# RaikoPipe/panda-gym

Hardware: AMD Instinct MI355X
Metric: aggregate env-steps/s, PandaReach 4096 envs @1 GPU; 1/2/4/8-GPU scaling (higher is better)
Workload: dtype f32; 1 GPU; PandaReach-v3 (ee control, sparse reward), 4096 envs per GPU, the reference's scene: table / plane contacts of the robot (BASELINE configs[1]); envs_per_gpu=4096, global_envs=4096, parallelism=env-sharded x1

## Files before the change

panda-gym_amd/csrc/pgx_kernels.hip:

```cpp
#include <hip/hip_runtime.h>
#include <math.h>
#include <stdint.h>

#include "../../include/pgx.h"
#include "pgx_default_model.h"
#include "pgx_common.h"
#include "pgx_dev.h"
#include "pgx_model_consts.h"
#include "pgx_rows.h"

#ifdef PGX_PROF
#define PGX_PROF_N 24
__device__ unsigned long long pgx_prof_counters[PGX_PROF_N];
#define PGX_PROF_WAVES 16384
__device__ unsigned long long pgx_prof_wave[PGX_PROF_WAVES][10];
extern "C" int pgx_prof_wave_read(unsigned long long* out, int n) {
    return (int)hipMemcpyFromSymbol(out, HIP_SYMBOL(pgx_prof_wave), sizeof(unsigned long long) * 10 * (size_t)n);
}
extern "C" int pgx_prof_read(unsigned long long* out, int clear) {
    hipError_t e = hipMemcpyFromSymbol(out, HIP_SYMBOL(pgx_prof_counters), sizeof(unsigned long long) * PGX_PROF_N);
    if (e == hipSuccess && clear) {
        unsigned long long z[PGX_PROF_N] = {0};
        e = hipMemcpyToSymbol(HIP_SYMBOL(pgx_prof_counters), z, sizeof z);
    }
// ... 2319 lines not shown
                PGX_PROF_SWEEP();
                if (resid <= res_thr || it + 1 >= n_it) break;
                resid = 0.0f;
#pragma unroll
                for (int r = 0; r < PGX_N_ROWS; r++)
                    if ((kPgxRowCode[r] >> 4) == 0) row(r, resid);
                limit_check();
                if (CONT && any_contact) contact_rows(resid);
                PGX_PROF_SWEEP();
                if (resid <= res_thr) break;
            }
            redo = __any(lmargin < 0.0f) || e.pgs_mode == 3;
            if (redo) {
                PGX_PROF_COUNT(12, 1);
#pragma unroll
                for (int j = 0; j < NJ; j++) dv[j] = L.spec0[j][ln];
                dvl = v3(L.spec0[NJ][ln], L.spec0[NJ + 1][ln], L.spec0[NJ + 2][ln]);
                dvw = v3(L.spec0[NJ + 3][ln], L.spec0[NJ + 4][ln], L.spec0[NJ + 5][ln]);
#pragma unroll
                for (int r = 0; r < PGX_N_ROWS; r++) lam[r] = 0.0f;
#pragma unroll
                for (int k = 0; k < CG; k++)
#pragma unroll
                    for (int dir = 0; dir < 3; dir++) {
                        lam0[k][dir] = (CONT && OBJ && k < n0) ? L.g0q[k][1 + dir][ln].w : 0.0f;
                        lam1[k][dir] = (CONT && k < n1) ? L.g1q[k][dir][5][ln].w : 0.0f;
                    }
            }
        } else {
            PGX_PROF_COUNT(13, 1);
        }
        for (int it = 0; redo && it < n_it; it += 2) {
            float resid = 0.0f;
#pragma unroll
            for (int r = PGX_N_ROWS - 1; r >= 0; r--) row(r, resid);
            if (CONT && any_contact) contact_rows(resid);
            PGX_PROF_SWEEP();
            if (resid <= res_thr || it + 1 >= n_it) break;
            resid = 0.0f;
#pragma unroll
            for (int r = 0; r < PGX_N_ROWS; r++) row(r, resid);
            if (CONT && any_contact) contact_rows(resid);
            PGX_PROF_SWEEP();
            if (resid <= res_thr) break;
        }
    }
#undef MINV
    PGX_PROF_SWEEPS_DONE();
    PGX_TRAP(4, n1, dv, NJ, m);
    PGX_PROF_MARK(4);
    PGX_PROF_COUNT(11, any_contact ? 1 : 0);
#pragma unroll
    for (int j = 0; j < NJ; j++) {
        float vn = fminf(fmaxf(vu[j] + dv[j], -m.max_vel), m.max_vel);
        qd[j] = vn;
        q[j] += m.dt * vn;
    }
    PGX_TRAP(5, n1, q, NJ, m);
    PGX_TRAP(6, n1, qd, NJ, m);
    if (CONT) {
        ContactLds& L = *Lp;
#pragma unroll
        for (int s = 0; s < CG; s++) {
            L.cache[2 * s][ln] = s < n0 ? L.g0id[s][ln] : -1.0f;
            L.cache[2 * s + 1][ln] = s < n0 ? lam0[s][0] : 0.0f;
            L.cache[8 + 2 * s][ln] = s < n1 ? L.g1id[s][ln] : -1.0f;
            L.cache[8 + 2 * s + 1][ln] = s < n1 ? lam1[s][0] : 0.0f;
        }
    }
    if (OBJ) object_integrate(m, ob, vcu + dvl, wcu + dvw);
    PGX_PROF_MARK(5);
}

constexpr bool limit_rows_paired() {
    for (int r = 0; r < NJ; r++)
        if ((kPgxRowCode[r] >> 4) != 0) return false;
    for (int r = NJ; r + 1 < PGX_N_ROWS; r += 2)
        if ((kPgxRowCode[r] >> 4) != 1 || (kPgxRowCode[r + 1] >> 4) != 2 ||
            (kPgxRowCode[r] & 15) != (kPgxRowCode[r + 1] & 15))
            return false;
    return (PGX_N_ROWS - NJ) % 2 == 0;
}

template <int OBJ, int CONT, int PART = 1, int AO = 0, int FULL = 0>
__device__ __forceinline__ bool substep_g(MPtr mp, const PgxDevEnv& e, float* q, float* qd, const float* tq,
                                          ObjState& ob, ContactLdsGT<OBJ, FULL>* Lp, int es, int c, const LaneK& K,
                                          bool check = false) {
    MRef m = *fresh(mp);
    constexpr bool LDS_LIM = OBJ;
    constexpr bool NO_PART = OBJ && PART == 2;
    constexpr bool PERS = CONT && FULL && (OBJ || (AO && AO_PERS));
    Dyn D;
    substep_dyn_g<OBJ, CONT, AO, FULL>(m, e, q, qd, ob, Lp, es, D, c, K, check);
    if constexpr (AO) {
        if (D.coll) return true;
    }
    const V3 (&z)[NJ] = D.z;
    const V3 (&o)[NJ] = D.o;
    float vu[NJ];
#pragma unroll
    for (int j = 0; j < NJ; j++) vu[j] = D.vu[j];
    V3 vcu = D.vcu, wcu = D.wcu;
    PGX_PROF_MARK(2);
    const bool arm = c < NJ;
    const float inv_m = e.obj_inv_mass, inv_i = e.obj_inv_inertia;
    float mcol[NJ];
#pragma unroll
    for (int d = 0; d < NJ; d++) mcol[d] = D.mcol[d];
    const float kobj = OBJ ? ((c >= 7 && c < 10) ? inv_m : ((c >= 10 && c < 13) ? inv_i : 0.0f)) : 0.0f;
    const float vu_c = pick_gen(vu, vcu, wcu);
    float gv = 0.0f;

    constexpr int P0 = OBJ ? CG : 0;
    constexpr int CGR = ContactLdsGT<OBJ, FULL>::CGR;
    constexpr int NP = P0 + (CONT ? CGR : 0);
    constexpr int RB = CONT ? ContactLdsGT<OBJ, FULL>::RB : CGR;
    constexpr int NQR = ContactLdsGT<OBJ, FULL>::NQR;
    constexpr int NC_ = OBJ ? 13 : NJ;
    constexpr int XSTEP = 1;
    int n1x = 0;
    int nxr = 0;
    float cJ[NP > 0 ? NP : 1][3], cR[NP > 0 ? NP : 1][3], crhs[NP > 0 ? NP : 1][3], cjinv[NP > 0 ? NP : 1][3];
    float cden[NP > 0 ? NP : 1][3], clam[NP > 0 ? NP : 1][3];
    float pmu[NP > 0 ? NP : 1];
    bool act[NP > 0 ? NP : 1];
    int n0 = 0, n1 = 0;
    if (CONT) {
        ContactLdsGT<OBJ, FULL>& L = *Lp;
        n0 = L.cnt[0][es];
        n1 = L.cnt[1][es];
        const float erp_dt = m.contact_erp * m.inv_dt;
        float cid0[CG], cim0[CG], cid1[CGR], cim1[CGR];
#pragma unroll
        for (int s2 = 0; s2 < CG; s2++) {
            cid0[s2] = OBJ ? L.cache[2 * s2][es] : -1.0f;
            cim0[s2] = OBJ ? L.cache[2 * s2 + 1][es] : 0.0f;
        }
#pragma unroll
        for (int s2 = 0; s2 < CGR; s2++) {
            cid1[s2] = L.cache[CACHE1 + 2 * s2][es];
            cim1[s2] = L.cache[CACHE1 + 2 * s2 + 1][es];
        }
        auto warm_of = [&](const float* ids, const float* ims, auto n_c, float id) __attribute__((always_inline)) {
            float w = 0.0f;
#pragma unroll
            for (int s2 = 0; s2 < decltype(n_c)::value; s2++) w = ids[s2] == id ? m.warmstart * ims[s2] : w;
            return w;
        };
#pragma unroll
        for (int p = 0; p < NP; p++) pmu[p] = m.friction;
#pragma unroll
        for (int k = 0; k < P0; k++) {
            act[k] = k < n0;
            const float4 r4 = L.g0q[k][0][es];
            const V3 r = v3(r4.x, r4.y, r4.z);
            const float id = L.g0id[k][es];
            const float warm = warm_of(cid0, cim0, IC<CG>{}, id);
            V3 nk = lds3(L.g0n[k], es), t1, t2;
            nk = act[k] ? nk : v3(0.0f, 0.0f, 1.0f);
            plane_space(nk, t1, t2);
#pragma unroll
            for (int dir = 0; dir < 3; dir++) {
                const V3 lin = dir == 0 ? nk : (dir == 1 ? t1 : t2);
                const V3 ang = cross(r, lin);
                const float den = inv_m + dot(ang, ang) * inv_i;
                const float jinv = den > 2.220446e-16f ? fast_rcp(den) : 0.0f;
// ... 228 lines not shown
                    w = fmaf(Jq[l], bcast16<l>(gv), w);
                });
                gwr = w;
            };
            build(IC<0>{}, Wm, Wc, gw);
            if constexpr (TWO) { if (g1k_any[1]) build(IC<1>{}, Wm2, Wc2, gw2); }
        }
    }
    constexpr int XB = (RB > CGR) ? (3 * (RB - CGR) + GW - 1) / GW : 1;
    float xs_rhs[XB], xs_lam[XB], xs_fk[XB], xs_jinv[XB];
    auto load_xs = [&](bool start) __attribute__((always_inline)) {
        if constexpr (RB > CGR) {
            ContactLdsGT<OBJ, FULL>& L = *Lp;
            __builtin_amdgcn_fence(__ATOMIC_SEQ_CST, "wavefront");
#pragma unroll
            for (int b = 0; b < XB; b++) {
                const int xq = GW * b + c;
                const bool ok = xq < 3 * nxr;
                const int xr = ok ? xq : 0;
                xs_lam[b] = ok ? L.xlam0[xr][es] : 0.0f;
                if (start) {
                    xs_rhs[b] = ok ? L.xrhs[xr][es] : 0.0f;
                    xs_fk[b] = ok ? L.xfk[xr][es] : 0.0f;
                    xs_jinv[b] = ok ? L.xjinv[xr][es] : 0.0f;
                }
            }
        }
    };
#pragma unroll
    for (int b = 0; b < XB; b++) { xs_rhs[b] = 0.0f; xs_lam[b] = 0.0f; xs_fk[b] = 0.0f; xs_jinv[b] = 0.0f; }
    if (RB > CGR && nxr > 0) load_xs(true);
    PGX_PROF_MARK(23);

    float den[NJ], jinv[NJ];
#pragma unroll
    for (int d = 0; d < NJ; d++) {
        den[d] = D.mdiag[d];
        jinv[d] = den[d] > 2.220446e-16f ? fast_rcp(den[d]) : 0.0f;
    }
    float rhs[PGX_N_ROWS];
#pragma unroll
    for (int r = 0; r < PGX_N_ROWS; r++) {
        const int kind = kPgxRowCode[r] >> 4, d = kPgxRowCode[r] & 15;
        rhs[r] = 0.0f;
        if (kind == 0) {
            const float pos_term = (tq[d] - q[d]) * m.inv_dt;
            const float desired = m.kp * pos_term + vu[d] + m.kd * (0.0f - vu[d]);
            rhs[r] = desired - vu[d];
        }
    }
    auto init_limit_rows = [&]() __attribute__((always_inline)) {
#pragma unroll
        for (int r = 0; r < PGX_N_ROWS; r++) {
            const int kind = kPgxRowCode[r] >> 4, d = kPgxRowCode[r] & 15;
            if (kind == 0) continue;
            const float rel = kind == 2 ? -vu[d] : vu[d];
            const float pen = kind == 1 ? (q[d] - kLower[d]) : (kUpper[d] - q[d]);
            float verr = -rel, perr = 0.0f;
            if (pen > 0.0f) verr -= pen * m.inv_dt;
            else perr = -pen * m.erp * m.inv_dt;
            rhs[r] = perr + verr;
        }
    };
    bool ok_c = true;
    bool far_nc = true;
    if (arm) {
        float B = 0.0f;
#pragma unroll
        for (int k = 0; k < NJ; k++) B += fabsf(mcol[k]) * m.max_impulse[k];
        B = B * 1.001f + 1e-6f;
        float lo_a[NJ], up_a[NJ];
#pragma unroll
        for (int d = 0; d < NJ; d++) { lo_a[d] = kLower[d]; up_a[d] = kUpper[d]; }
        const float qc = pick_arm(q, 0.0f);
        const float penl = qc - pick_arm(lo_a, 0.0f), penu = pick_arm(up_a, 0.0f) - qc;
        ok_c = penl > 0.0f && penu > 0.0f && (vu_c - B) > -penl * m.inv_dt && (vu_c + B) < penu * m.inv_dt;
    }
    far_nc = !row_any(!ok_c);
    const bool far = far_nc && n1 == 0;
    float mcs[NJ], wms[NJ], wms2[NJ];
    constexpr int PK = AO ? PGX_PK_AO : PGX_PK;
    constexpr bool PKM = WROWS && (PK & 1) != 0, PKC = WROWS && (PK & 2) != 0;
    constexpr bool PKD = TWO && FULL && !PKM && !PKC && (PK & 4) != 0;
    f2 mw[NJ], crw[NQ], mw2[NJ], cw2[NQ];
    f2 bnd[NJ];
    float lam[PGX_N_ROWS], lhi[NJ];
#pragma unroll
    for (int d = 0; d < NJ; d++) {
        mcs[d] = mcol[d] * jinv[d];
        wms[d] = Wm[d] * jinv[d];
        wms2[d] = Wm2[d] * jinv[d];
        lhi[d] = m.limit_max_imp * den[d];
    }
    auto init_bounds = [&]() __attribute__((always_inline)) {
#pragma unroll
        for (int r = 0; r < PGX_N_ROWS; r++) {
            const int kind = kPgxRowCode[r] >> 4, d = kPgxRowCode[r] & 15;
            lam[r] = 0.0f;
            if (kind == 0) bnd[d] = (f2){-m.max_impulse[d] * den[d], m.max_impulse[d] * den[d]};
            else if (LDS_LIM) __hip_atomic_store(&Lp->llam[r - NJ][es], 0.0f, __ATOMIC_RELAXED, __HIP_MEMORY_SCOPE_WAVEFRONT);
        }
    };
    init_bounds();
    auto mrow = [&](auto rc, auto g2_c, float& resid) __attribute__((always_inline)) {
        constexpr int r = decltype(rc)::value;
        constexpr int kind = kPgxRowCode[r] >> 4, d = kPgxRowCode[r] & 15;
        const float x = kind == 2 ? rhs[r] + bcast16<d>(gv) : rhs[r] - bcast16<d>(gv);
        float delta;
        if constexpr (kind == 0) {
            delta = __builtin_amdgcn_fmed3f(x, bnd[d].x, bnd[d].y);
            bnd[d] -= (f2){delta, delta};
        } else if constexpr (LDS_LIM) {
            float* lr = &Lp->lrhs[r - NJ][es];
            float* ll = &Lp->llam[r - NJ][es];
            const float rr = __hip_atomic_load(lr, __ATOMIC_RELAXED, __HIP_MEMORY_SCOPE_WAVEFRONT);
            const float lm = __hip_atomic_load(ll, __ATOMIC_RELAXED, __HIP_MEMORY_SCOPE_WAVEFRONT);
            const float xl = kind == 2 ? rr + bcast16<d>(gv) : rr - bcast16<d>(gv);
            delta = __builtin_amdgcn_fmed3f(xl, -lm, lhi[d] - lm);
            __hip_atomic_store(ll, lm + delta, __ATOMIC_RELAXED, __HIP_MEMORY_SCOPE_WAVEFRONT);
        } else {
            delta = __builtin_amdgcn_fmed3f(x, -lam[r], lhi[d] - lam[r]);
            lam[r] += delta;
        }
        const float sd = kind == 2 ? -delta : delta;
        if constexpr (PKD) {
            gv += mcs[d] * sd;
            if constexpr (decltype(g2_c)::value) pk_fma_acc(gw, gw2, mw2[d], sd);
            else gw += mw2[d].x * sd;
        } else {
            if constexpr (PKM) {
                pk_fma_acc(gv, gw, mw[d], sd);
            } else {
                gv += mcs[d] * sd;
                if constexpr (WROWS) gw += wms[d] * sd;
            }
            if constexpr (TWO && decltype(g2_c)::value) gw2 += wms2[d] * sd;
        }
        resid = fmaxf(resid, fabsf(delta));
    };
    constexpr int NPP = NP > 0 ? NP : 1;
    float fk[NPP][3];
    bool rok[NPP][3];
#pragma unroll
    for (int p = 0; p < NP; p++)
#pragma unroll
        for (int dir = 0; dir < 3; dir++) {
            rok[p][dir] = act[p] && cjinv[p][dir] != 0.0f;
            fk[p][dir] = rok[p][dir] ? pmu[p] * cjinv[p][0] * cden[p][dir] : 0.0f;
            crhs[p][dir] *= cden[p][dir];
            clam[p][dir] *= cden[p][dir];
            cR[p][dir] *= cjinv[p][dir];
        }
    if constexpr (WROWS) {
#pragma unroll
        for (int q = 0; q < NQ; q++) {
            Wc[q] *= cjinv[q / 3][q % 3];
            if (TWO) Wc2[q] *= cjinv[q / 3][q % 3];
        }
        float r0 = 0.0f, r1 = 0.0f;
        sfor<0, NQ>([&](auto qc) __attribute__((always_inline)) {
            constexpr int q = decltype(qc)::value;
            if constexpr (q < GW) r0 = lane_sel<q>(crhs[q / 3][q % 3], r0);
            else r1 = lane_sel<q - GW>(crhs[q / 3][q % 3], r1);
        });
        gw = r0 - gw;
        if (TWO) gw2 = r1 - gw2;
        if constexpr (OBJ) {
            sfor<0, NQ / 3>([&](auto pc) __attribute__((always_inline)) {
                constexpr int p = decltype(pc)::value, q = 3 * p;
                const bool usable = act[p] && cjinv[p][0] != 0.0f;
                if constexpr (q < GW) gw = usable ? gw : lane_sel<q>(-3.0e38f, gw);
                else gw2 = usable ? gw2 : lane_sel<q - GW>(-3.0e38f, gw2);
            });
        }
#pragma unroll
        for (int q = 0; q < NQ; q++) { Wc[q] = -Wc[q]; Wc2[q] = -Wc2[q]; }
#pragma unroll
        for (int d = 0; d < NJ; d++) { wms[d] = -wms[d]; wms2[d] = -wms2[d]; }
        if constexpr (PKM) {
#pragma unroll
            for (int d = 0; d < NJ; d++) mw[d] = (f2){mcs[d], wms[d]};
        }
        if constexpr (PKC) {
#pragma unroll
            for (int q = 0; q < NQ; q++) crw[q] = (f2){cR[q / 3][q % 3], Wc[q]};
        }
        if constexpr (PKD) {
#pragma unroll
            for (int d = 0; d < NJ; d++) mw2[d] = (f2){wms[d], wms2[d]};
#pragma unroll
            for (int q = 0; q < NQ; q++) cw2[q] = (f2){Wc[q], Wc2[q]};
        }
    }
    float chi[NPP];
    if constexpr (CONT) {
#pragma unroll
        for (int p = 0; p < NP; p++) Lp->pjn[p][es] = cjinv[p][0];
    }
#pragma unroll
    for (int p = 0; p < NP; p++) {
        chi[p] = rok[p][0] ? 3.0e38f : 0.0f;
        if (WROWS && !rok[p][0]) clam[p][0] = 0.0f;
    }
    auto crow = [&](auto pc, auto dc, const bool fr, auto g2_c, float& resid) __attribute__((always_inline)) {
        constexpr int p = decltype(pc)::value, dir = decltype(dc)::value, q = 3 * p + dir;
        const float ln_n = clam[p][0], lm = clam[p][dir];
        float lo, hi;
        if (fr) {
            const float mk = ln_n > 0.0f ? 1.0f : 0.0f;
            const float fkv = fk[p][dir];
            const f2 b = ((f2){-fkv, fkv} * ln_n - lm) * mk;
            lo = b.x;
            hi = b.y;
        } else {
            lo = -lm;
            hi = OBJ ? 3.0e38f : chi[p];
        }
        const float x = q < GW ? bcast16<q % GW>(gw) : bcast16<q % GW>(gw2);
        const float delta = __builtin_amdgcn_fmed3f(x, lo, hi);
        clam[p][dir] = lm + delta;
        if constexpr (PKD) {
            gv += cR[p][dir] * delta;
            if constexpr (decltype(g2_c)::value) pk_fma_acc(gw, gw2, cw2[q], delta);
            else gw += cw2[q].x * delta;
        } else {
            if constexpr (PKC) {
                pk_fma_acc(gv, gw, crw[q], delta);
            } else {
                gv += cR[p][dir] * delta;
                gw += Wc[q] * delta;
            }
            if constexpr (TWO && decltype(g2_c)::value) gw2 += Wc2[q] * delta;
        }
        resid = fmaxf(resid, fabsf(delta));
    };
    int n1w = 0;
#pragma unroll
    for (int k = 0; k < CGR; k++) n1w = g1k_any[k] ? k + 1 : n1w;
    n1w = __builtin_amdgcn_readfirstlane(n1w);
    const bool g0_any = CONT && OBJ && __any(n0 > 0);
    const bool g1_any = CONT && __any(n1 > 0);
    int rcol = c;
    auto extra_rows = [&](auto fr_c, auto nx_c, auto g2_c, float& resid) __attribute__((always_inline)) {
        constexpr int FR = decltype(fr_c)::value, NX = decltype(nx_c)::value;
        if constexpr (WROWS && RB > CGR && NX > 0) {
            ContactLdsGT<OBJ, FULL>& L = *Lp;
            const float gvb = gv;
            sfor<0, NX>([&](auto kc) __attribute__((always_inline)) {
                constexpr int kx = decltype(kc)::value;
                sfor<FR ? 1 : 0, FR ? 3 : 1>([&](auto dc) __attribute__((always_inline)) {
                    constexpr int dir = decltype(dc)::value, xq = 3 * kx + dir;
                    constexpr int b = xq / GW, l = xq % GW, bn = (3 * kx) / GW, ln_ = (3 * kx) % GW;
                    const float J = L.xd[es][xq][c].x;
                    const float Rs = L.xd[es][xq][rcol].y;
                    const float w = sum16(J * gv);
                    const float lm = bcast16<l>(xs_lam[b]), fkv = bcast16<l>(xs_fk[b]);
                    float lo, hi;
                    if constexpr (dir != 0) {
                        const float ln_n = bcast16<ln_>(xs_lam[bn]);
                        const float mk = ln_n > 0.0f ? 1.0f : 0.0f;
                        const f2 bb = ((f2){-fkv, fkv} * ln_n - lm) * mk;
                        lo = bb.x;
                        hi = bb.y;
                    } else {
                        lo = -lm;
                        hi = fkv;
                    }
                    const float delta = __builtin_amdgcn_fmed3f(bcast16<l>(xs_rhs[b]) - w, lo, hi);
                    xs_lam[b] = lane_sel<l>(lm + delta, xs_lam[b]);
                    gv += Rs * delta;
                    resid = fmaxf(resid, fabsf(delta));
                });
            });
            const float dgv = gv - gvb;
            auto correct = [&](auto reg_c, float& gwr) __attribute__((always_inline)) {
                constexpr int R0 = decltype(reg_c)::value * GW;
                const int qr = R0 + c < NQR ? R0 + c : NQR - 1;
                const float4* jrow = &L.wJ[es][qr][0];
                float Jq[NC];
#pragma unroll
                for (int v4 = 0; v4 < (NC + 3) / 4; v4++) {
                    const float4 t = jrow[v4];
                    const float tv[4] = {t.x, t.y, t.z, t.w};
#pragma unroll
                    for (int u = 0; u < 4; u++)
                        if (4 * v4 + u < NC) Jq[4 * v4 + u] = tv[u];
                }
                float d = Jq[0] * bcast16<0>(dgv);
                sfor<1, NC>([&](auto lc) __attribute__((always_inline)) {
                    constexpr int l2 = decltype(lc)::value;
                    d = fmaf(Jq[l2], bcast16<l2>(dgv), d);
                });
                gwr -= R0 + c < NQR ? d : 0.0f;
            };
            correct(IC<0>{}, gw);
            if constexpr (TWO && decltype(g2_c)::value) correct(IC<1>{}, gw2);
        }
    };
    auto contact_rows = [&](auto nw_c, auto nx_c, auto g2_c, float& resid) __attribute__((always_inline)) {
        constexpr int NW = decltype(nw_c)::value;
#pragma unroll
        for (int fr = 0; fr < 2; fr++) {
            if (OBJ && g0_any) {
                sfor<0, P0>([&](auto kc) __attribute__((always_inline)) {
                    if (fr) { crow(kc, IC<1>{}, true, g2_c, resid); crow(kc, IC<2>{}, true, g2_c, resid); }
                    else crow(kc, IC<0>{}, false, g2_c, resid);
                });
            }
            if (NW < 0 && !g1_any) continue;
            sfor<0, (CONT ? (NW >= 0 ? NW : CGR) : 0)>([&](auto kc) __attribute__((always_inline)) {
                constexpr int k = decltype(kc)::value;
                if (NW >= 0 || k < n1w) {
                    if (fr) {
                        crow(IC<P0 + k>{}, IC<1>{}, true, g2_c, resid);
                        crow(IC<P0 + k>{}, IC<2>{}, true, g2_c, resid);
                    } else {
                        crow(IC<P0 + k>{}, IC<0>{}, false, g2_c, resid);
                    }
                }
            });
            if (fr) extra_rows(IC<1>{}, nx_c, g2_c, resid);
            else extra_rows(IC<0>{}, nx_c, g2_c, resid);
        }
    };
    const bool any_contact = CONT && __any(n0 > 0 || n1 > 0);
    const int n_it = m.num_iterations;
    float res_thr = m.residual_abs;
    asm("" : "+s"(res_thr));
    PGX_PROF_MARK(3);
    PGX_PROF_COUNT(9, 1);
    PGX_PROF_SWEEPS_DECL;
    float rl_c = -1.0f, ru_c = -1.0f;
    float lmargin = 3.0e38f;
    auto limit_check = [&]() __attribute__((always_inline)) {
        lmargin = fminf(lmargin, fminf(gv - rl_c, -(ru_c + gv)));
    };
    constexpr int KMAX = CONT ? 1 : 2;
    constexpr int SL0 = OBJ ? 13 : NJ;
    unsigned dmask = 0u;
    float smcs[KMAX], swms[KMAX], swms2[KMAX], srh[KMAX][2], slhi[KMAX], slam[KMAX][2];
    f2 smw[KMAX];
    auto srow = [&](auto sc, auto kc, auto g2_c, float& resid) __attribute__((always_inline)) {
        constexpr int S = decltype(sc)::value, KIND = decltype(kc)::value;
        const float x = KIND == 2 ? srh[S][1] + bcast16<SL0 + S>(gv) : srh[S][0] - bcast16<SL0 + S>(gv);
        const float delta = __builtin_amdgcn_fmed3f(x, -slam[S][KIND - 1], slhi[S] - slam[S][KIND - 1]);
        slam[S][KIND - 1] += delta;
        const float sd = KIND == 2 ? -delta : delta;
        if constexpr (PKM) {
            pk_fma_acc(gv, gw, smw[S], sd);
        } else {
            gv += smcs[S] * sd;
            if constexpr (WROWS) gw += swms[S] * sd;
        }
        if constexpr (TWO && decltype(g2_c)::value) gw2 += swms2[S] * sd;
        resid = fmaxf(resid, fabsf(delta));
    };
    static_assert(limit_rows_paired(), "limit rows come as (lower, upper) pairs of one dof after the motor rows");
    auto solve = [&](auto mode_c, auto nw_c, auto k_c, auto nx_c) __attribute__((always_inline)) {
        constexpr int MODE = decltype(mode_c)::value;
        constexpr int NW = decltype(nw_c)::value;
        constexpr int K = decltype(k_c)::value;
        constexpr bool G2 = TWO && (NW < 0 || 3 * (P0 + NW) > GW);
        const IC<G2 ? 1 : 0> g2_c{};
        for (int it = 0; it < n_it; it += 2) {
            float resid = 0.0f;
            if constexpr (MODE == 1 || MODE == 3) limit_check();
            if constexpr (MODE == 3) {
                sfor<0, K>([&](auto i) __attribute__((always_inline)) {
                    constexpr int S = K - 1 - decltype(i)::value;
                    srow(IC<S>{}, IC<2>{}, g2_c, resid);
                    srow(IC<S>{}, IC<1>{}, g2_c, resid);
                    limit_check();
                });
            }
            sfor<0, PGX_N_ROWS>([&](auto i) __attribute__((always_inline)) {
                constexpr int r = PGX_N_ROWS - 1 - decltype(i)::value;
                if constexpr (MODE == 2 || (kPgxRowCode[r] >> 4) == 0) mrow(IC<r>{}, g2_c, resid);
            });
            if (CONT && (OBJ || NW > 0 || (NW < 0 && any_contact))) contact_rows(nw_c, nx_c, g2_c, resid);
            PGX_PROF_SWEEP();
            if (resid <= res_thr || it + 1 >= n_it) break;
            resid = 0.0f;
            sfor<0, PGX_N_ROWS>([&](auto i) __attribute__((always_inline)) {
                constexpr int r = decltype(i)::value;
                if constexpr (MODE == 2 || (kPgxRowCode[r] >> 4) == 0) mrow(IC<r>{}, g2_c, resid);
            });
            if constexpr (MODE == 1 || MODE == 3) limit_check();
            if constexpr (MODE == 3) {
                sfor<0, K>([&](auto sc) __attribute__((always_inline)) {
                    srow(sc, IC<1>{}, g2_c, resid);
                    srow(sc, IC<2>{}, g2_c, resid);
                    limit_check();
                });
            }
            if (CONT && (OBJ || NW > 0 || (NW < 0 && any_contact))) contact_rows(nw_c, nx_c, g2_c, resid);
            PGX_PROF_SWEEP();
            if (resid <= res_thr) break;
        }
    };
    auto solve_w = [&](auto mode_c, auto k_c) __attribute__((always_inline)) {
        constexpr int MODE = decltype(mode_c)::value;
        if constexpr (WROWS) {
            if (n1w == 0) solve(mode_c, IC<0>{}, k_c, IC<0>{});
            else if (nxr == 0 && n1w <= 2) solve(mode_c, IC<2>{}, k_c, IC<0>{});
            else if (CGR > 4 && nxr == 0 && n1w <= 4) solve(mode_c, IC<(CGR > 4 ? 4 : CGR)>{}, k_c, IC<0>{});
            else if constexpr (RB > CGR && MODE != 3) {
                if (nxr == 0) {
                    solve(mode_c, IC<CGR>{}, k_c, IC<0>{});
                } else {
                    sfor<1, (RB - CGR) / XSTEP + 1>([&](auto ic) __attribute__((always_inline)) {
                        constexpr int NXC = decltype(ic)::value * XSTEP;
                        if (nxr == NXC) solve(mode_c, IC<CGR>{}, k_c, IC<NXC>{});
                    });
                }
            } else {
                solve(mode_c, IC<CGR>{}, k_c, IC<0>{});
            }
        } else {
            solve(mode_c, IC<-1>{}, k_c, IC<0>{});
        }
    };
#ifndef PGX_NO_PARK_SOLVE
    constexpr bool PARK_SOLVE = CONT && (OBJ || AO || PART == 2);
#else
    constexpr bool PARK_SOLVE = false;
#endif
    auto park = [&](int k, float v) __attribute__((always_inline)) {
        __hip_atomic_store(&Lp->psv[k][es], v, __ATOMIC_RELAXED, __HIP_MEMORY_SCOPE_WAVEFRONT);
    };
    auto unpark = [&](int k) __attribute__((always_inline)) {
        return __hip_atomic_load(&Lp->psv[k][es], __ATOMIC_RELAXED, __HIP_MEMORY_SCOPE_WAVEFRONT);
    };
    if constexpr (PARK_SOLVE) {
#pragma unroll
        for (int j = 0; j < NJ; j++) { park(j, q[j]); park(NJ + j, vu[j]); }
        if constexpr (OBJ) {
            park(14, ob.p.x); park(15, ob.p.y); park(16, ob.p.z);
            park(17, ob.qx); park(18, ob.qy); park(19, ob.qz); park(20, ob.qw);
            park(21, vcu.x); park(22, vcu.y); park(23, vcu.z);
            park(24, wcu.x); park(25, wcu.y); park(26, wcu.z);
        }
    }
    if (__all(far)) {
        solve(IC<0>{}, IC<0>{}, IC<0>{}, IC<0>{});
    } else {
        PGX_PROF_COUNT(10, 1);
        init_limit_rows();
        if constexpr (LDS_LIM) {
#pragma unroll
            for (int r = NJ; r < PGX_N_ROWS; r++)
                __hip_atomic_store(&Lp->lrhs[r - NJ][es], rhs[r], __ATOMIC_RELAXED, __HIP_MEMORY_SCOPE_WAVEFRONT);
        }
        if (e.pgs_mode != 2) {
            float rl[NJ], ru[NJ];
#pragma unroll
            for (int r = NJ; r < PGX_N_ROWS; r++) {
                const int kind = kPgxRowCode[r] >> 4, d = kPgxRowCode[r] & 15;
                if (kind == 1) rl[d] = rhs[r];
                else ru[d] = rhs[r];
            }
            rl_c = pick_arm(rl, -3.0e38f);
            ru_c = pick_arm(ru, -3.0e38f);
            const bool spec_all = __all(far_nc);
            int nk = 0;
            if (!spec_all) {
                const uint64_t bm = __ballot(arm && !ok_c);
                dmask = __builtin_amdgcn_readfirstlane((unsigned)((bm | (bm >> 16) | (bm >> 32) | (bm >> 48)) & 0x7Fu));
                nk = __builtin_popcount(dmask);
            }
            const float gv0 = gv, gw0 = gw, gw20 = gw2;
            if constexpr (CONT) {
#pragma unroll
                for (int p = 0; p < NP; p++) Lp->pl0[p][es] = clam[p][0];
            }
            if (PART && !NO_PART && !spec_all && nk <= KMAX && nxr == 0) {
                PGX_PROF_COUNT(7, 1);
                int ds[2] = {0, 0};
                int k = 0;
                sfor<0, (PGX_N_ROWS - NJ) / 2>([&](auto pc) __attribute__((always_inline)) {
                    constexpr int d = kPgxRowCode[NJ + 2 * decltype(pc)::value] & 15;
                    if ((dmask >> d) & 1u) { if (k == 0) ds[0] = d; else ds[1] = d; k++; }
                });
                ds[0] = __builtin_amdgcn_readfirstlane(ds[0]);
                ds[1] = __builtin_amdgcn_readfirstlane(ds[1]);
                const int src = (int)(threadIdx.x & ~(unsigned)(GW - 1));
                auto mirror = [&](float& x) __attribute__((always_inline)) {
                    x = lane_sel<SL0>(__shfl(x, src + ds[0]), x);
                    if (KMAX > 1 && nk > 1) x = lane_sel<SL0 + 1>(__shfl(x, src + ds[1]), x);
                };
#pragma unroll
                for (int d = 0; d < NJ; d++) {
                    if constexpr (PKM) {
                        float t = mw[d].x;
                        mirror(t);
                        mw[d].x = t;
                    } else {
                        mirror(mcs[d]);
                    }
                }
                mirror(gv);
                if (g1_any) {
#pragma unroll
                    for (int p = 0; p < NP; p++)
#pragma unroll
                        for (int dir = 0; dir < 3; dir++) {
                            if constexpr (PKC) {
                                float t = crw[3 * p + dir].x;
                                mirror(t);
                                crw[3 * p + dir].x = t;
                            } else {
                                mirror(cR[p][dir]);
                            }
                        }
                }
#pragma unroll
                for (int S = 0; S < KMAX; S++) {
                    if constexpr (PKM) smw[S] = mw[0];
                    else { smcs[S] = mcs[0]; swms[S] = PKD ? mw2[0].x : wms[0]; }
                    swms2[S] = PKD ? mw2[0].y : wms2[0]; slhi[S] = lhi[0];
                    srh[S][0] = rl[0]; srh[S][1] = ru[0];
                    slam[S][0] = 0.0f; slam[S][1] = 0.0f;
                    sfor<1, NJ>([&](auto dc) __attribute__((always_inline)) {
                        constexpr int d = decltype(dc)::value;
                        const bool hit = ds[S] == d;
                        auto sel = [&](float a, float o) __attribute__((always_inline)) { return hit ? a : o; };
                        if constexpr (PKM) smw[S] = hit ? mw[d] : smw[S];
                        else { smcs[S] = sel(mcs[d], smcs[S]); swms[S] = sel(PKD ? mw2[d].x : wms[d], swms[S]); }
                        swms2[S] = sel(PKD ? mw2[d].y : wms2[d], swms2[S]);
                        slhi[S] = sel(lhi[d], slhi[S]);
                        srh[S][0] = sel(rl[d], srh[S][0]); srh[S][1] = sel(ru[d], srh[S][1]);
                    });
                }
                if ((dmask >> c) & 1u) { rl_c = -3.0e38f; ru_c = -3.0e38f; }
                if (c == SL0) rcol = ds[0];
                if (KMAX > 1 && nk > 1 && c == SL0 + 1) rcol = ds[1];
                PGX_PROF_COUNT(16, nk == 2 ? 1 : 0);
                PGX_PROF_COUNT(18, any_contact ? 1 : 0);
                if (KMAX == 1 || nk == 1) solve_w(IC<3>{}, IC<1>{});
                else solve_w(IC<3>{}, IC<KMAX>{});
            } else if (spec_all) {
                solve_w(IC<1>{}, IC<0>{});
            } else {
                lmargin = -1.0f;
            }
            const bool viol = lmargin < 0.0f;
            if (__any(row_any(viol)) || e.pgs_mode == 3) {
                PGX_PROF_COUNT(12, 1);
                gv = gv0;
                gw = gw0;
                gw2 = gw20;
#pragma unroll
                for (int p = 0; p < NP; p++) {
                    clam[p][0] = CONT ? Lp->pl0[p][es] : 0.0f;
                    clam[p][1] = 0.0f;
                    clam[p][2] = 0.0f;
                }
                if (RB > CGR && nxr > 0) load_xs(false);
                init_bounds();
                solve_w(IC<2>{}, IC<0>{});
            }
        } else {
            PGX_PROF_COUNT(13, 1);
            solve_w(IC<2>{}, IC<0>{});
        }
    }
    PGX_PROF_SWEEPS_DONE();
    PGX_PROF_MARK(4);
    PGX_PROF_COUNT(11, any_contact ? 1 : 0);
    if constexpr (PARK_SOLVE) {
#pragma unroll
        for (int j = 0; j < NJ; j++) { q[j] = unpark(j); vu[j] = unpark(NJ + j); }
        if constexpr (OBJ) {
            ob.p = v3(unpark(14), unpark(15), unpark(16));
            ob.qx = unpark(17); ob.qy = unpark(18); ob.qz = unpark(19); ob.qw = unpark(20);
            vcu = v3(unpark(21), unpark(22), unpark(23));
            wcu = v3(unpark(24), unpark(25), unpark(26));
        }
    }
    sfor<0, NJ>([&](auto jc) __attribute__((always_inline)) {
        constexpr int j = decltype(jc)::value;
        const float vn = fminf(fmaxf(vu[j] + bcast16<j>(gv), -m.max_vel), m.max_vel);
        qd[j] = vn;
        q[j] += m.dt * vn;
    });
    if (CONT) {
        ContactLdsGT<OBJ, FULL>& L = *Lp;
        float gid0[CG], pj0[CG], gid1[CGR], pj1[CGR];
#pragma unroll
        for (int s = 0; s < CG; s++) {
            gid0[s] = OBJ ? L.g0id[s][es] : -1.0f;
            pj0[s] = OBJ ? L.pjn[s][es] : 0.0f;
        }
#pragma unroll
        for (int s = 0; s < CGR; s++) {
            gid1[s] = L.g1id[s][es];
            pj1[s] = L.pjn[P0 + s][es];
        }
#pragma unroll
        for (int s = 0; s < CG; s++) {
            L.cache[2 * s][es] = (OBJ && s < n0) ? gid0[s] : -1.0f;
            L.cache[2 * s + 1][es] = (OBJ && s < n0) ? clam[s][0] * pj0[s] : 0.0f;
        }
#pragma unroll
        for (int s = 0; s < CGR; s++) {
            L.cache[CACHE1 + 2 * s][es] = s < n1 ? gid1[s] : -1.0f;
            L.cache[CACHE1 + 2 * s + 1][es] = s < n1 ? clam[P0 + s][0] * pj1[s] : 0.0f;
        }
        if constexpr (RB > CGR) {
            if (n1x > CGR) {
#pragma unroll
                for (int b = 0; b < XB; b++)
                    if (GW * b + c < 3 * (n1x - CGR)) L.xlam[GW * b + c][es] = xs_lam[b];
                __builtin_amdgcn_fence(__ATOMIC_SEQ_CST, "wavefront");
            }
            for (int s = CGR; s < RB; s++) {
                const int xq = 3 * (s - CGR);
                L.cache[CACHE1 + 2 * s][es] = s < n1 ? L.g1id[s][es] : -1.0f;
                L.cache[CACHE1 + 2 * s + 1][es] = s < n1 ? L.xlam[xq][es] * L.xjinv[xq][es] : 0.0f;
            }
        }
        if constexpr (PERS) {
            static_assert(RB <= GW, "one lane per robot slot");
            __builtin_amdgcn_fence(__ATOMIC_SEQ_CST, "wavefront");
            if (c < n1) {
                const int w = L.g1w[c][es];
                if (w >= 0) L.mimp[w][es] = L.cache[CACHE1 + 2 * c + 1][es];
            }
        }
    }
    if (OBJ) {
        const V3 dvl = v3(bcast16<7>(gv), bcast16<8>(gv), bcast16<9>(gv));
        const V3 dvw = v3(bcast16<10>(gv), bcast16<11>(gv), bcast16<12>(gv));
        object_integrate(m, ob, vcu + dvl, wcu + dvw);
    }
    PGX_PROF_MARK(5);
    return false;
}

__device__ __forceinline__ void ee_state(MRef m, const float* q, const float* qd, V3& pos, V3& vel) {
    Chain k;
    fk_chain(m, q, k);
    pos = k.o[NJ - 1] + mulc(k.R[NJ - 1], kEeCom);
    V3 vv = v3(0, 0, 0);
#pragma unroll
    for (int j = 0; j < NJ; j++) vv = vv + qd[j] * cross(col(k.R[j], 2), pos - k.o[j]);
    vel = vv;
// ... 1279 lines not shown
```

Baseline: 11.20 million env-steps/s.

## Merge contact-row gradient into upper lanes of motor gradient register in PGS solve

```diff
diff --git a/panda-gym_amd/csrc/pgx_kernels.hip b/panda-gym_amd/csrc/pgx_kernels.hip
--- a/panda-gym_amd/csrc/pgx_kernels.hip
+++ b/panda-gym_amd/csrc/pgx_kernels.hip
@@ -2425,6 +2425,13 @@
     return (PGX_N_ROWS - NJ) % 2 == 0;
 }
 
+constexpr int last_motor_row() {
+    int r = 0;
+    for (int i = 0; i < PGX_N_ROWS; i++)
+        if ((kPgxRowCode[i] >> 4) == 0) r = i;
+    return r;
+}
+
 template <int OBJ, int CONT, int PART = 1, int AO = 0, int FULL = 0>
 __device__ __forceinline__ bool substep_g(MPtr mp, const PgxDevEnv& e, float* q, float* qd, const float* tq,
                                           ObjState& ob, ContactLdsGT<OBJ, FULL>* Lp, int es, int c, const LaneK& K,
@@ -2819,6 +2826,15 @@
     constexpr int PK = AO ? PGX_PK_AO : PGX_PK;
     constexpr bool PKM = WROWS && (PK & 1) != 0, PKC = WROWS && (PK & 2) != 0;
     constexpr bool PKD = TWO && FULL && !PKM && !PKC && (PK & 4) != 0;
+    constexpr bool MERGE = WROWS && !OBJ && !AO && !PKM && !PKC && PART != 2;
+    constexpr int MG0 = 8;
+    static_assert(!MERGE || MG0 + 6 <= GW, "6 contact rows from lane MG0");
+    auto hi_sel = [&](float a, float other) __attribute__((always_inline)) {
+        float r;
+        asm("v_cndmask_b32 %0, %1, %2, %3" : "=v"(r) : "v"(other), "v"(a), "s"(0xFF00FF00FF00FF00ull));
+        return r;
+    };
+    auto ror8 = [&](float v) __attribute__((always_inline)) { return dpp<0x128>(v); };
     f2 mw[NJ], crw[NQ], mw2[NJ], cw2[NQ];
     f2 bnd[NJ];
     float lam[PGX_N_ROWS], lhi[NJ];
@@ -2839,7 +2855,7 @@
         }
     };
     init_bounds();
-    auto mrow = [&](auto rc, auto g2_c, float& resid) __attribute__((always_inline)) {
+    auto mrow = [&](auto rc, auto g2_c, auto mg_c, float& resid) __attribute__((always_inline)) {
         constexpr int r = decltype(rc)::value;
         constexpr int kind = kPgxRowCode[r] >> 4, d = kPgxRowCode[r] & 15;
         const float x = kind == 2 ? rhs[r] + bcast16<d>(gv) : rhs[r] - bcast16<d>(gv);
@@ -2860,7 +2876,9 @@
             lam[r] += delta;
         }
         const float sd = kind == 2 ? -delta : delta;
-        if constexpr (PKD) {
+        if constexpr (decltype(mg_c)::value) {
+            gv += mcs[d] * sd;
+        } else if constexpr (PKD) {
             gv += mcs[d] * sd;
             if constexpr (decltype(g2_c)::value) pk_fma_acc(gw, gw2, mw2[d], sd);
             else gw += mw2[d].x * sd;
@@ -2873,7 +2891,8 @@
             }
             if constexpr (TWO && decltype(g2_c)::value) gw2 += wms2[d] * sd;
         }
-        resid = fmaxf(resid, fabsf(delta));
+        if constexpr (decltype(mg_c)::value == 2) resid = fabsf(delta);
+        else resid = fmaxf(resid, fabsf(delta));
     };
     constexpr int NPP = NP > 0 ? NP : 1;
     float fk[NPP][3];
@@ -2939,7 +2958,7 @@
         chi[p] = rok[p][0] ? 3.0e38f : 0.0f;
         if (WROWS && !rok[p][0]) clam[p][0] = 0.0f;
     }
-    auto crow = [&](auto pc, auto dc, const bool fr, auto g2_c, float& resid) __attribute__((always_inline)) {
+    auto crow = [&](auto pc, auto dc, const bool fr, auto g2_c, auto mg_c, float& resid) __attribute__((always_inline)) {
         constexpr int p = decltype(pc)::value, dir = decltype(dc)::value, q = 3 * p + dir;
         const float ln_n = clam[p][0], lm = clam[p][dir];
         float lo, hi;
@@ -2953,10 +2972,14 @@
             lo = -lm;
             hi = OBJ ? 3.0e38f : chi[p];
         }
-        const float x = q < GW ? bcast16<q % GW>(gw) : bcast16<q % GW>(gw2);
+        constexpr bool MG = decltype(mg_c)::value != 0;
+        const float x = MG ? bcast16<(MG0 + q) % GW>(gv)
+                           : (q < GW ? bcast16<q % GW>(gw) : bcast16<q % GW>(gw2));
         const float delta = __builtin_amdgcn_fmed3f(x, lo, hi);
         clam[p][dir] = lm + delta;
-        if constexpr (PKD) {
+        if constexpr (MG) {
+            gv += cR[p][dir] * delta;
+        } else if constexpr (PKD) {
             gv += cR[p][dir] * delta;
             if constexpr (decltype(g2_c)::value) pk_fma_acc(gw, gw2, cw2[q], delta);
             else gw += cw2[q].x * delta;
@@ -2969,7 +2992,8 @@
             }
             if constexpr (TWO && decltype(g2_c)::value) gw2 += Wc2[q] * delta;
         }
-        resid = fmaxf(resid, fabsf(delta));
+        if constexpr (decltype(mg_c)::value == 2) resid = fabsf(delta);
+        else resid = fmaxf(resid, fabsf(delta));
     };
     int n1w = 0;
 #pragma unroll
@@ -3034,14 +3058,14 @@
             if constexpr (TWO && decltype(g2_c)::value) correct(IC<1>{}, gw2);
         }
     };
-    auto contact_rows = [&](auto nw_c, auto nx_c, auto g2_c, float& resid) __attribute__((always_inline)) {
+    auto contact_rows = [&](auto nw_c, auto nx_c, auto g2_c, auto mg_c, float& resid) __attribute__((always_inline)) {
         constexpr int NW = decltype(nw_c)::value;
 #pragma unroll
         for (int fr = 0; fr < 2; fr++) {
             if (OBJ && g0_any) {
                 sfor<0, P0>([&](auto kc) __attribute__((always_inline)) {
-                    if (fr) { crow(kc, IC<1>{}, true, g2_c, resid); crow(kc, IC<2>{}, true, g2_c, resid); }
-                    else crow(kc, IC<0>{}, false, g2_c, resid);
+                    if (fr) { crow(kc, IC<1>{}, true, g2_c, mg_c, resid); crow(kc, IC<2>{}, true, g2_c, mg_c, resid); }
+                    else crow(kc, IC<0>{}, false, g2_c, mg_c, resid);
                 });
             }
             if (NW < 0 && !g1_any) continue;
@@ -3049,10 +3073,10 @@
                 constexpr int k = decltype(kc)::value;
                 if (NW >= 0 || k < n1w) {
                     if (fr) {
-                        crow(IC<P0 + k>{}, IC<1>{}, true, g2_c, resid);
-                        crow(IC<P0 + k>{}, IC<2>{}, true, g2_c, resid);
+                        crow(IC<P0 + k>{}, IC<1>{}, true, g2_c, mg_c, resid);
+                        crow(IC<P0 + k>{}, IC<2>{}, true, g2_c, mg_c, resid);
                     } else {
-                        crow(IC<P0 + k>{}, IC<0>{}, false, g2_c, resid);
+                        crow(IC<P0 + k>{}, IC<0>{}, false, g2_c, mg_c, resid);
                     }
                 }
             });
@@ -3074,87 +3098,119 @@
     };
     constexpr int KMAX = CONT ? 1 : 2;
     constexpr int SL0 = OBJ ? 13 : NJ;
+    static_assert(!MERGE || SL0 + KMAX <= MG0, "the slot lanes (mirror() writes SL0 .. SL0 + KMAX - 1) end below the merged contact lanes");
+    static_assert((kPgxRowCode[0] >> 4) == 0, "row 0 is a motor row (the first row of a forward sweep)");
     unsigned dmask = 0u;
     float smcs[KMAX], swms[KMAX], swms2[KMAX], srh[KMAX][2], slhi[KMAX], slam[KMAX][2];
     f2 smw[KMAX];
-    auto srow = [&](auto sc, auto kc, auto g2_c, float& resid) __attribute__((always_inline)) {
+    auto srow = [&](auto sc, auto kc, auto g2_c, auto mg_c, float& resid) __attribute__((always_inline)) {
         constexpr int S = decltype(sc)::value, KIND = decltype(kc)::value;
         const float x = KIND == 2 ? srh[S][1] + bcast16<SL0 + S>(gv) : srh[S][0] - bcast16<SL0 + S>(gv);
         const float delta = __builtin_amdgcn_fmed3f(x, -slam[S][KIND - 1], slhi[S] - slam[S][KIND - 1]);
         slam[S][KIND - 1] += delta;
         const float sd = KIND == 2 ? -delta : delta;
-        if constexpr (PKM) {
+        if constexpr (decltype(mg_c)::value) {
+            gv += smcs[S] * sd;
+        } else if constexpr (PKM) {
             pk_fma_acc(gv, gw, smw[S], sd);
         } else {
             gv += smcs[S] * sd;
             if constexpr (WROWS) gw += swms[S] * sd;
         }
         if constexpr (TWO && decltype(g2_c)::value) gw2 += swms2[S] * sd;
-        resid = fmaxf(resid, fabsf(delta));
+        if constexpr (decltype(mg_c)::value == 2) resid = fabsf(delta);
+        else resid = fmaxf(resid, fabsf(delta));
     };
     static_assert(limit_rows_paired(), "limit rows come as (lower, upper) pairs of one dof after the motor rows");
-    auto solve = [&](auto mode_c, auto nw_c, auto k_c, auto nx_c) __attribute__((always_inline)) {
+    auto solve = [&](auto mode_c, auto nw_c, auto k_c, auto nx_c, auto mg_c) __attribute__((always_inline)) {
         constexpr int MODE = decltype(mode_c)::value;
         constexpr int NW = decltype(nw_c)::value;
         constexpr int K = decltype(k_c)::value;
         constexpr bool G2 = TWO && (NW < 0 || 3 * (P0 + NW) > GW);
         const IC<G2 ? 1 : 0> g2_c{};
+        constexpr bool MG = decltype(mg_c)::value != 0;
+        const IC<MG ? 2 : 0> mgf_c{};
+        constexpr int LASTM = last_motor_row();
         for (int it = 0; it < n_it; it += 2) {
             float resid = 0.0f;
             if constexpr (MODE == 1 || MODE == 3) limit_check();
             if constexpr (MODE == 3) {
                 sfor<0, K>([&](auto i) __attribute__((always_inline)) {
                     constexpr int S = K - 1 - decltype(i)::value;
-                    srow(IC<S>{}, IC<2>{}, g2_c, resid);
-                    srow(IC<S>{}, IC<1>{}, g2_c, resid);
+                    if constexpr (MG && S == K - 1) srow(IC<S>{}, IC<2>{}, g2_c, mgf_c, resid);
+                    else srow(IC<S>{}, IC<2>{}, g2_c, mg_c, resid);
+                    srow(IC<S>{}, IC<1>{}, g2_c, mg_c, resid);
                     limit_check();
                 });
             }
             sfor<0, PGX_N_ROWS>([&](auto i) __attribute__((always_inline)) {
                 constexpr int r = PGX_N_ROWS - 1 - decltype(i)::value;
-                if constexpr (MODE == 2 || (kPgxRowCode[r] >> 4) == 0) mrow(IC<r>{}, g2_c, resid);
+                if constexpr (MG && MODE != 3 && r == LASTM) mrow(IC<r>{}, g2_c, mgf_c, resid);
+                else if constexpr (MODE == 2 || (kPgxRowCode[r] >> 4) == 0) mrow(IC<r>{}, g2_c, mg_c, resid);
             });
-            if (CONT && (OBJ || NW > 0 || (NW < 0 && any_contact))) contact_rows(nw_c, nx_c, g2_c, resid);
+            if (CONT && (OBJ || NW > 0 || (NW < 0 && any_contact))) contact_rows(nw_c, nx_c, g2_c, mg_c, resid);
             PGX_PROF_SWEEP();
             if (resid <= res_thr || it + 1 >= n_it) break;
             resid = 0.0f;
             sfor<0, PGX_N_ROWS>([&](auto i) __attribute__((always_inline)) {
                 constexpr int r = decltype(i)::value;
-                if constexpr (MODE == 2 || (kPgxRowCode[r] >> 4) == 0) mrow(IC<r>{}, g2_c, resid);
+                if constexpr (MG && r == 0) mrow(IC<r>{}, g2_c, mgf_c, resid);
+                else if constexpr (MODE == 2 || (kPgxRowCode[r] >> 4) == 0) mrow(IC<r>{}, g2_c, mg_c, resid);
             });
             if constexpr (MODE == 1 || MODE == 3) limit_check();
             if constexpr (MODE == 3) {
                 sfor<0, K>([&](auto sc) __attribute__((always_inline)) {
-                    srow(sc, IC<1>{}, g2_c, resid);
-                    srow(sc, IC<2>{}, g2_c, resid);
+                    srow(sc, IC<1>{}, g2_c, mg_c, resid);
+                    srow(sc, IC<2>{}, g2_c, mg_c, resid);
                     limit_check();
                 });
             }
-            if (CONT && (OBJ || NW > 0 || (NW < 0 && any_contact))) contact_rows(nw_c, nx_c, g2_c, resid);
+            if (CONT && (OBJ || NW > 0 || (NW < 0 && any_contact))) contact_rows(nw_c, nx_c, g2_c, mg_c, resid);
             PGX_PROF_SWEEP();
             if (resid <= res_thr) break;
         }
     };
-    auto solve_w = [&](auto mode_c, auto k_c) __attribute__((always_inline)) {
+    const bool mg = MERGE && e.pgs_mode != 4 && n1w >= 1 && n1w <= 2 && nxr == 0;
+    auto merge_rows = [&]() __attribute__((always_inline)) {
+        if constexpr (MERGE) {
+#pragma unroll
+            for (int d = 0; d < NJ; d++) mcs[d] = hi_sel(ror8(wms[d]), mcs[d]);
+#pragma unroll
+            for (int q = 0; q < 6; q++) cR[q / 3][q % 3] = hi_sel(ror8(Wc[q]), cR[q / 3][q % 3]);
+            gv = hi_sel(ror8(gw), gv);
+        }
+    };
+    auto split_rows = [&]() __attribute__((always_inline)) {
+        if constexpr (MERGE) {
+#pragma unroll
+            for (int d = 0; d < NJ; d++) wms[d] = hi_sel(0.0f, ror8(mcs[d]));
+#pragma unroll
+            for (int q = 0; q < 6; q++) Wc[q] = hi_sel(0.0f, ror8(cR[q / 3][q % 3]));
+        }
+    };
+    auto solve_w = [&](auto mode_c, auto k_c, auto mgi_c) __attribute__((always_inline)) {
         constexpr int MODE = decltype(mode_c)::value;
-        if constexpr (WROWS) {
-            if (n1w == 0) solve(mode_c, IC<0>{}, k_c, IC<0>{});
-            else if (nxr == 0 && n1w <= 2) solve(mode_c, IC<2>{}, k_c, IC<0>{});
-            else if (CGR > 4 && nxr == 0 && n1w <= 4) solve(mode_c, IC<(CGR > 4 ? 4 : CGR)>{}, k_c, IC<0>{});
+        const IC<0> m0{};
+        if constexpr (decltype(mgi_c)::value) {
+            solve(mode_c, IC<2>{}, k_c, IC<0>{}, IC<(MODE != 2) ? 1 : 0>{});
+        } else if constexpr (WROWS) {
+            if (n1w == 0) solve(mode_c, IC<0>{}, k_c, IC<0>{}, m0);
+            else if (nxr == 0 && n1w <= 2) solve(mode_c, IC<2>{}, k_c, IC<0>{}, m0);
+            else if (CGR > 4 && nxr == 0 && n1w <= 4) solve(mode_c, IC<(CGR > 4 ? 4 : CGR)>{}, k_c, IC<0>{}, m0);
             else if constexpr (RB > CGR && MODE != 3) {
                 if (nxr == 0) {
-                    solve(mode_c, IC<CGR>{}, k_c, IC<0>{});
+                    solve(mode_c, IC<CGR>{}, k_c, IC<0>{}, m0);
                 } else {
                     sfor<1, (RB - CGR) / XSTEP + 1>([&](auto ic) __attribute__((always_inline)) {
                         constexpr int NXC = decltype(ic)::value * XSTEP;
-                        if (nxr == NXC) solve(mode_c, IC<CGR>{}, k_c, IC<NXC>{});
+                        if (nxr == NXC) solve(mode_c, IC<CGR>{}, k_c, IC<NXC>{}, m0);
                     });
                 }
             } else {
-                solve(mode_c, IC<CGR>{}, k_c, IC<0>{});
+                solve(mode_c, IC<CGR>{}, k_c, IC<0>{}, m0);
             }
         } else {
-            solve(mode_c, IC<-1>{}, k_c, IC<0>{});
+            solve(mode_c, IC<-1>{}, k_c, IC<0>{}, m0);
         }
     };
 #ifndef PGX_NO_PARK_SOLVE
@@ -3179,7 +3235,7 @@
         }
     }
     if (__all(far)) {
-        solve(IC<0>{}, IC<0>{}, IC<0>{}, IC<0>{});
+        solve(IC<0>{}, IC<0>{}, IC<0>{}, IC<0>{}, IC<0>{});
     } else {
         PGX_PROF_COUNT(10, 1);
         init_limit_rows();
@@ -3210,95 +3266,19 @@
 #pragma unroll
                 for (int p = 0; p < NP; p++) Lp->pl0[p][es] = clam[p][0];
             }
-            if (PART && !NO_PART && !spec_all && nk <= KMAX && nxr == 0) {
-                PGX_PROF_COUNT(7, 1);
-                int ds[2] = {0, 0};
-                int k = 0;
-                sfor<0, (PGX_N_ROWS - NJ) / 2>([&](auto pc) __attribute__((always_inline)) {
-                    constexpr int d = kPgxRowCode[NJ + 2 * decltype(pc)::value] & 15;
-                    if ((dmask >> d) & 1u) { if (k == 0) ds[0] = d; else ds[1] = d; k++; }
-                });
-                ds[0] = __builtin_amdgcn_readfirstlane(ds[0]);
-                ds[1] = __builtin_amdgcn_readfirstlane(ds[1]);
-                const int src = (int)(threadIdx.x & ~(unsigned)(GW - 1));
-                auto mirror = [&](float& x) __attribute__((always_inline)) {
-                    x = lane_sel<SL0>(__shfl(x, src + ds[0]), x);
-                    if (KMAX > 1 && nk > 1) x = lane_sel<SL0 + 1>(__shfl(x, src + ds[1]), x);
+            if constexpr (MERGE) {
+                auto limit_solves = [&](auto mgi_c) __attribute__((always_inline)) {
+#include "pgx_limit_solves.inc"
                 };
-#pragma unroll
-                for (int d = 0; d < NJ; d++) {
-                    if constexpr (PKM) {
-                        float t = mw[d].x;
-                        mirror(t);
-                        mw[d].x = t;
-                    } else {
-                        mirror(mcs[d]);
-                    }
-                }
-                mirror(gv);
-                if (g1_any) {
-#pragma unroll
-                    for (int p = 0; p < NP; p++)
-#pragma unroll
-                        for (int dir = 0; dir < 3; dir++) {
-                            if constexpr (PKC) {
-                                float t = crw[3 * p + dir].x;
-                                mirror(t);
-                                crw[3 * p + dir].x = t;
-                            } else {
-                                mirror(cR[p][dir]);
-                            }
-                        }
-                }
-#pragma unroll
-                for (int S = 0; S < KMAX; S++) {
-                    if constexpr (PKM) smw[S] = mw[0];
-                    else { smcs[S] = mcs[0]; swms[S] = PKD ? mw2[0].x : wms[0]; }
-                    swms2[S] = PKD ? mw2[0].y : wms2[0]; slhi[S] = lhi[0];
-                    srh[S][0] = rl[0]; srh[S][1] = ru[0];
-                    slam[S][0] = 0.0f; slam[S][1] = 0.0f;
-                    sfor<1, NJ>([&](auto dc) __attribute__((always_inline)) {
-                        constexpr int d = decltype(dc)::value;
-                        const bool hit = ds[S] == d;
-                        auto sel = [&](float a, float o) __attribute__((always_inline)) { return hit ? a : o; };
-                        if constexpr (PKM) smw[S] = hit ? mw[d] : smw[S];
-                        else { smcs[S] = sel(mcs[d], smcs[S]); swms[S] = sel(PKD ? mw2[d].x : wms[d], swms[S]); }
-                        swms2[S] = sel(PKD ? mw2[d].y : wms2[d], swms2[S]);
-                        slhi[S] = sel(lhi[d], slhi[S]);
-                        srh[S][0] = sel(rl[d], srh[S][0]); srh[S][1] = sel(ru[d], srh[S][1]);
-                    });
-                }
-                if ((dmask >> c) & 1u) { rl_c = -3.0e38f; ru_c = -3.0e38f; }
-                if (c == SL0) rcol = ds[0];
-                if (KMAX > 1 && nk > 1 && c == SL0 + 1) rcol = ds[1];
-                PGX_PROF_COUNT(16, nk == 2 ? 1 : 0);
-                PGX_PROF_COUNT(18, any_contact ? 1 : 0);
-                if (KMAX == 1 || nk == 1) solve_w(IC<3>{}, IC<1>{});
-                else solve_w(IC<3>{}, IC<KMAX>{});
-            } else if (spec_all) {
-                solve_w(IC<1>{}, IC<0>{});
+                if (mg) limit_solves(IC<1>{});
+                else limit_solves(IC<0>{});
             } else {
-                lmargin = -1.0f;
-            }
-            const bool viol = lmargin < 0.0f;
-            if (__any(row_any(viol)) || e.pgs_mode == 3) {
-                PGX_PROF_COUNT(12, 1);
-                gv = gv0;
-                gw = gw0;
-                gw2 = gw20;
-#pragma unroll
-                for (int p = 0; p < NP; p++) {
-                    clam[p][0] = CONT ? Lp->pl0[p][es] : 0.0f;
-                    clam[p][1] = 0.0f;
-                    clam[p][2] = 0.0f;
-                }
-                if (RB > CGR && nxr > 0) load_xs(false);
-                init_bounds();
-                solve_w(IC<2>{}, IC<0>{});
+                const IC<0> mgi_c{};
+#include "pgx_limit_solves.inc"
             }
         } else {
             PGX_PROF_COUNT(13, 1);
-            solve_w(IC<2>{}, IC<0>{});
+            solve_w(IC<2>{}, IC<0>{}, IC<0>{});
         }
     }
     PGX_PROF_SWEEPS_DONE();
diff --git a/panda-gym_amd/csrc/pgx_limit_solves.inc b/panda-gym_amd/csrc/pgx_limit_solves.inc
--- /dev/null
+++ b/panda-gym_amd/csrc/pgx_limit_solves.inc
@@ -0,0 +1,96 @@
+            constexpr bool MGI = decltype(mgi_c)::value != 0;
+            if constexpr (MGI) merge_rows();
+            const float gm0 = gv;
+            if (PART && !NO_PART && !spec_all && nk <= KMAX && nxr == 0) {
+                PGX_PROF_COUNT(7, 1);
+                int ds[2] = {0, 0};
+                int k = 0;
+                sfor<0, (PGX_N_ROWS - NJ) / 2>([&](auto pc) __attribute__((always_inline)) {
+                    constexpr int d = kPgxRowCode[NJ + 2 * decltype(pc)::value] & 15;
+                    if ((dmask >> d) & 1u) { if (k == 0) ds[0] = d; else ds[1] = d; k++; }
+                });
+                ds[0] = __builtin_amdgcn_readfirstlane(ds[0]);
+                ds[1] = __builtin_amdgcn_readfirstlane(ds[1]);
+                const int src = (int)(threadIdx.x & ~(unsigned)(GW - 1));
+                auto mirror = [&](float& x) __attribute__((always_inline)) {
+                    x = lane_sel<SL0>(__shfl(x, src + ds[0]), x);
+                    if (KMAX > 1 && nk > 1) x = lane_sel<SL0 + 1>(__shfl(x, src + ds[1]), x);
+                };
+#pragma unroll
+                for (int d = 0; d < NJ; d++) {
+                    if constexpr (PKM) {
+                        float t = mw[d].x;
+                        mirror(t);
+                        mw[d].x = t;
+                    } else {
+                        mirror(mcs[d]);
+                    }
+                }
+                mirror(gv);
+                if (g1_any) {
+#pragma unroll
+                    for (int p = 0; p < NP; p++)
+#pragma unroll
+                        for (int dir = 0; dir < 3; dir++) {
+                            if constexpr (PKC) {
+                                float t = crw[3 * p + dir].x;
+                                mirror(t);
+                                crw[3 * p + dir].x = t;
+                            } else {
+                                mirror(cR[p][dir]);
+                            }
+                        }
+                }
+#pragma unroll
+                for (int S = 0; S < KMAX; S++) {
+                    if constexpr (PKM) smw[S] = mw[0];
+                    else { smcs[S] = mcs[0]; if constexpr (!MGI) swms[S] = PKD ? mw2[0].x : wms[0]; }
+                    if constexpr (!MGI) swms2[S] = PKD ? mw2[0].y : wms2[0];
+                    slhi[S] = lhi[0];
+                    srh[S][0] = rl[0]; srh[S][1] = ru[0];
+                    slam[S][0] = 0.0f; slam[S][1] = 0.0f;
+                    sfor<1, NJ>([&](auto dc) __attribute__((always_inline)) {
+                        constexpr int d = decltype(dc)::value;
+                        const bool hit = ds[S] == d;
+                        auto sel = [&](float a, float o) __attribute__((always_inline)) { return hit ? a : o; };
+                        if constexpr (PKM) smw[S] = hit ? mw[d] : smw[S];
+                        else { smcs[S] = sel(mcs[d], smcs[S]); if constexpr (!MGI) swms[S] = sel(PKD ? mw2[d].x : wms[d], swms[S]); }
+                        if constexpr (!MGI) swms2[S] = sel(PKD ? mw2[d].y : wms2[d], swms2[S]);
+                        slhi[S] = sel(lhi[d], slhi[S]);
+                        srh[S][0] = sel(rl[d], srh[S][0]); srh[S][1] = sel(ru[d], srh[S][1]);
+                    });
+                }
+                if ((dmask >> c) & 1u) { rl_c = -3.0e38f; ru_c = -3.0e38f; }
+                if (c == SL0) rcol = ds[0];
+                if (KMAX > 1 && nk > 1 && c == SL0 + 1) rcol = ds[1];
+                PGX_PROF_COUNT(16, nk == 2 ? 1 : 0);
+                PGX_PROF_COUNT(18, any_contact ? 1 : 0);
+                if (KMAX == 1 || nk == 1) solve_w(IC<3>{}, IC<1>{}, mgi_c);
+                else solve_w(IC<3>{}, IC<KMAX>{}, mgi_c);
+            } else if (spec_all) {
+                solve_w(IC<1>{}, IC<0>{}, mgi_c);
+            } else {
+                lmargin = -1.0f;
+            }
+            const bool viol = lmargin < 0.0f;
+            if (__any(row_any(viol)) || e.pgs_mode == 3) {
+                PGX_PROF_COUNT(12, 1);
+                if constexpr (MGI) {
+                    split_rows();
+                    gv = gm0;
+                    gw = hi_sel(0.0f, ror8(gm0));
+                } else {
+                    gv = gv0;
+                    gw = gw0;
+                    gw2 = gw20;
+                }
+#pragma unroll
+                for (int p = 0; p < NP; p++) {
+                    clam[p][0] = CONT ? Lp->pl0[p][es] : 0.0f;
+                    clam[p][1] = 0.0f;
+                    clam[p][2] = 0.0f;
+                }
+                if (RB > CGR && nxr > 0) load_xs(false);
+                init_bounds();
+                solve_w(IC<2>{}, IC<0>{}, mgi_c);
+            }
```

After: 11.65 million env-steps/s (median of 6 runs). 4.0% higher.
